# kakaobrain/rq-vae-transformer

Measured on NVIDIA H100. Metric: 256x256 images/sec (ImageNet 1.4B RQ-Transformer, 8x8x4 codes, K=16384, top-k 1024, sample+decode), higher is better.
Workload: dtype fp16

## Files before the change

rq-vae-transformer_b200/csrc/conv_tc.cu:

```cuda
#include <cstdlib>

#include "kernels.h"
#include "tc_common.cuh"

namespace rqb {

struct ConvTcParams {
    int B, H, W, Cin, Cout;
    int ks;
    int stride;
    int TW, TH, NB;
    int tiles_x, tiles_y, tiles_b, n_tiles_n;
    const float* bias;
    const float* residual;
    float* out;
    int out_nchw;
    void* out16;
    int gelu, fmt;
    int64_t m_rows;
    double* gn_part;
    int gn_chunks;
};

constexpr int CT_THREADS = 288;
// ... 222 lines not shown
    const int grid = total < n_sm ? total : n_sm;
    conv_tc_kernel<BN, STAGES, PASSES><<<grid, CT_THREADS, smem, st>>>(tmA, tmB, tmAlo, tmBlo, p);
    return check_launch("conv_tc");
}

constexpr int C3_HALO_BYTES = 10 * 10 * 2 * 128;

template <int BN>
__device__ __forceinline__ void c3_mma_kblock(float (&acc)[BN / 2], uint32_t a, uint32_t b, bool first) {
    constexpr int B_BYTES = BN * 64 * 2;
    constexpr uint32_t SBO = 10 * 128;
#pragma unroll
    for (int j = 0; j < 4; j++)
        tc::Wgmma<BN, 0>::mma(acc, tc::gmma_desc_k128(a + C3_HALO_BYTES + j * 32, SBO), tc::gmma_desc_k128(b + j * 32),
                              (!first || j > 0) ? 1u : 0u);
#pragma unroll
    for (int j = 0; j < 4; j++)
        tc::Wgmma<BN, 0>::mma(acc, tc::gmma_desc_k128(a + j * 32, SBO), tc::gmma_desc_k128(b + B_BYTES + j * 32), 1u);
#pragma unroll
    for (int j = 0; j < 4; j++)
        tc::Wgmma<BN, 0>::mma(acc, tc::gmma_desc_k128(a + j * 32, SBO), tc::gmma_desc_k128(b + j * 32), 1u);
}

template <int BM, int STAGES, int SLOT_BYTES, int HALO_BYTES>
__device__ __forceinline__ void c3_produce(const CUtensorMap* tmA, const CUtensorMap* tmB, const CUtensorMap* tmAlo, const CUtensorMap* tmBlo,
                                           const ConvTcParams& p, uint8_t* smem, uint8_t* wst, uint64_t* full, uint64_t* empty,
                                           uint64_t* hfull, uint64_t* hempty) {
    constexpr int NOPS = 2;
    constexpr int B_BYTES = BM * 64 * 2;
    constexpr int STAGE_BYTES = NOPS * B_BYTES;
    const int cslabs = p.Cin / 64;
    const int total = p.tiles_x * p.tiles_y * p.tiles_b * p.n_tiles_n;
    const uint32_t halo_tx = NOPS * 10 * (p.TH + 2) * p.NB * 128;
    uint32_t it = 0, hit = 0;
    for (int tile = blockIdx.x; tile < total; tile += gridDim.x) {
        const int nt = tile % p.n_tiles_n, mt = tile / p.n_tiles_n;
        const int tx = mt % p.tiles_x, ty = (mt / p.tiles_x) % p.tiles_y, tb = mt / (p.tiles_x * p.tiles_y);
        const int x0 = tx * 8, y0 = ty * p.TH, b0 = tb * p.NB;
        for (int sl = 0; sl < cslabs; sl++, hit++) {
            const int c0 = sl * 64;
            for (int tap = 0; tap < 9; tap++, it++) {
                const int s = it % STAGES;
                tc::mbar_wait(&empty[s], ((it / STAGES) & 1) ^ 1);
                tc::mbar_expect_tx(&full[s], STAGE_BYTES);
                uint8_t* w = wst + s * STAGE_BYTES;
                tc::tma_load_2d(w, tmB, &full[s], tap * p.Cin + c0, nt * BM, tc::L2_EVICT_LAST);
                tc::tma_load_2d(w + B_BYTES, tmBlo, &full[s], tap * p.Cin + c0, nt * BM, tc::L2_EVICT_LAST);
                if (tap == 0) {
                    const int h = hit % 2;
                    tc::mbar_wait(&hempty[h], ((hit / 2) & 1) ^ 1);
                    tc::mbar_expect_tx(&hfull[h], halo_tx);
                    uint8_t* a = smem + h * SLOT_BYTES;
                    tc::tma_load_4d(a, tmA, &hfull[h], c0, x0 - 1, y0 - 1, b0, tc::L2_EVICT_NORMAL);
                    tc::tma_load_4d(a + HALO_BYTES, tmAlo, &hfull[h], c0, x0 - 1, y0 - 1, b0, tc::L2_EVICT_NORMAL);
                }
            }
        }
    }
}

template <int BN, int STAGES>
__global__ void __launch_bounds__(CT_THREADS, 1)
conv3x3_tc_kernel(const __grid_constant__ CUtensorMap tmA, const __grid_constant__ CUtensorMap tmB,
                  const __grid_constant__ CUtensorMap tmAlo, const __grid_constant__ CUtensorMap tmBlo, ConvTcParams p) {
    constexpr int B_BYTES = BN * 64 * 2;
    constexpr int NOPS = 2;
    constexpr int HSLOTS = 2;
    constexpr int SLOT_BYTES = NOPS * C3_HALO_BYTES;
    constexpr int STAGE_BYTES = NOPS * B_BYTES;
    constexpr int CW = BN < 32 ? BN : 32;
// ... 98 lines not shown
template <int TH, int NB>
__device__ __forceinline__ void c3w_mma_kblock(float (&acc)[C3wTile<TH, NB>::NP / 2], const uint32_t (&fh)[4][4],
                                               const uint32_t (&fl)[4][4], uint32_t x, bool first) {
    constexpr int NI = C3wTile<TH, NB>::NI, HALO = C3wTile<TH, NB>::HALO;
    constexpr uint32_t SBO = 10 * 128, IMG = (TH + 2) * 10 * 128;
    auto mma = [&acc](const uint32_t (&a)[4], uint32_t xa, uint32_t accumulate) {
#pragma unroll
        for (int b = 0; b < NB; b++)
            tc::WgmmaRA<NI>::mma(*reinterpret_cast<float(*)[NI / 2]>(&acc[b * (NI / 2)]), a, tc::gmma_desc_k128(xa + b * IMG, SBO),
                                 accumulate);
    };
#pragma unroll
    for (int j = 0; j < 4; j++) mma(fh[j], x + HALO + j * 32, (!first || j > 0) ? 1u : 0u);
#pragma unroll
    for (int j = 0; j < 4; j++) mma(fl[j], x + j * 32, 1u);
#pragma unroll
    for (int j = 0; j < 4; j++) mma(fh[j], x + j * 32, 1u);
}

__device__ __forceinline__ void ldsm_x4(uint32_t (&r)[4], uint32_t addr) {
    asm volatile("ldmatrix.sync.aligned.m8n8.x4.shared.b16 {%0,%1,%2,%3}, [%4];" : "=r"(r[0]), "=r"(r[1]), "=r"(r[2]), "=r"(r[3]) : "r"(addr));
}

template <int TH, int NB, int STAGES>
__global__ void __launch_bounds__(C3W_THREADS, 1)
conv3x3_wreg_kernel(const __grid_constant__ CUtensorMap tmA, const __grid_constant__ CUtensorMap tmB,
                    const __grid_constant__ CUtensorMap tmAlo, const __grid_constant__ CUtensorMap tmBlo, ConvTcParams p) {
    using T = C3wTile<TH, NB>;
    constexpr int NOPS = 2;
    constexpr int SLOT_BYTES = NOPS * T::HALO;
    constexpr int B_BYTES = 128 * 128;
    constexpr int STAGE_BYTES = NOPS * B_BYTES;
    extern __shared__ uint8_t smem_raw[];
    uint8_t* smem = reinterpret_cast<uint8_t*>((reinterpret_cast<uintptr_t>(smem_raw) + 1023) & ~uintptr_t(1023));
    uint8_t* wst = smem + 2 * SLOT_BYTES;
    float* stage = reinterpret_cast<float*>(wst + STAGES * STAGE_BYTES);
    float2* gnred = reinterpret_cast<float2*>(stage + 32 * C3W_SP);
    uint64_t* full = reinterpret_cast<uint64_t*>(gnred + 256);
    uint64_t* empty = full + STAGES;
    uint64_t* hfull = empty + STAGES;
    uint64_t* hempty = hfull + 2;

    const int warp = threadIdx.x >> 5, lane = threadIdx.x & 31;
    const int nkb = 9 * (p.Cin / 64);
    const int total = p.tiles_x * p.tiles_y * p.tiles_b * p.n_tiles_n;

    if (warp == 8 && lane == 0) {
        tc::prefetch_tmap(&tmA);
        tc::prefetch_tmap(&tmB);
        for (int s = 0; s < STAGES; s++) { tc::mbar_init(&full[s], 1); tc::mbar_init(&empty[s], 8); }
        for (int h = 0; h < 2; h++) { tc::mbar_init(&hfull[h], 1); tc::mbar_init(&hempty[h], 8); }
        tc::fence_barrier_init();
    }
    __syncthreads();

    if (warp >= 8) {
        tc::setmaxnreg_dec<C3W_REGS_PRODUCER>();
        if (warp == 8 && lane == 0)
            c3_produce<128, STAGES, SLOT_BYTES, T::HALO>(&tmA, &tmB, &tmAlo, &tmBlo, p, smem, wst, full, empty, hfull, hempty);
        return;
    }
    tc::setmaxnreg_inc<C3W_REGS_CONSUMER>();

    const int wg = warp >> 2;
    const uint32_t lofs = (64 * wg + 16 * (warp & 3) + (lane & 7) + 8 * ((lane >> 3) & 1)) * 128 + (((lane >> 4) ^ (lane & 7)) << 4);
    const uint32_t halo0 = tc::smem_u32(smem), wst0 = tc::smem_u32(wst);

    float acc[T::NP / 2];
#pragma unroll
    for (int i = 0; i < T::NP / 2; i++) acc[i] = 0.f;
    uint32_t frag[2][2][4][4];
    uint32_t it = 0, hit = 0;
    auto kblock = [&](int kb, uint32_t (&fr)[2][4][4]) {
        const int tap = kb % 9;
        if (tap == 0) tc::mbar_wait(&hfull[hit % 2], (hit / 2) & 1);
        const int s = it % STAGES;
        tc::mbar_wait(&full[s], (it / STAGES) & 1);
        const uint32_t w = wst0 + s * STAGE_BYTES + lofs;
#pragma unroll
        for (int j = 0; j < 4; j++) {
            ldsm_x4(fr[0][j], w ^ (32 * j));
            ldsm_x4(fr[1][j], (w + B_BYTES) ^ (32 * j));
        }
        const uint32_t x = halo0 + (hit % 2) * SLOT_BYTES + ((tap / 3) * 10 + tap % 3) * 128;
        tc::wgmma_fence();
        c3w_mma_kblock<TH, NB>(acc, fr[0], fr[1], x, kb == 0);
        tc::wgmma_commit();
        __syncwarp();
        if (lane == 0) tc::mbar_arrive(&empty[s]);
        tc::wgmma_wait<1>();
        if (tap == 0 && kb > 0 && lane == 0) tc::mbar_arrive(&hempty[(hit - 1) % 2]);
        it++;
        if (tap == 8) hit++;
    };
    for (int tile = blockIdx.x; tile < total; tile += gridDim.x) {
        for (int kb = 0; kb < nkb; kb += 2) {
            kblock(kb, frag[0]);
            if (kb + 1 < nkb) kblock(kb + 1, frag[1]);
        }
        tc::wgmma_wait<0>();
        tc::acc_fence(acc);
        if (lane == 0) tc::mbar_arrive(&hempty[(hit - 1) % 2]);

        const int nt = tile % p.n_tiles_n, mt = tile / p.n_tiles_n;
        const int tx = mt % p.tiles_x, ty = (mt / p.tiles_x) % p.tiles_y, tb = mt / (p.tiles_x * p.tiles_y);
        const int srow = 2 * (lane & 3), scol = 64 * wg + 16 * (warp & 3) + (lane >> 2);
        const int n0 = nt * 128 + 4 * lane;
#pragma unroll
        for (int c = 0; c < T::NP / 32; c++) {
#pragma unroll
            for (int jj = 0; jj < 4; jj++)
#pragma unroll
                for (int i = 0; i < 4; i++)
                    stage[(8 * jj + srow + (i & 1)) * C3W_SP + scol + 8 * (i >> 1)] = acc[4 * (4 * c + jj) + i];
            tc::bar_sync(1, 256);
            const int x = tx * 8 + warp, y0 = ty * TH + (4 * c) % TH, b = tb * NB + (4 * c) / TH;
            const int64_t off = (((int64_t)b * p.H + y0) * p.W + x) * p.Cout + n0;
            const int rs = p.W * p.Cout;
            const float4 bb = *reinterpret_cast<const float4*>(p.bias + n0);
            float4 v[4];
            unsigned valid = 0;
#pragma unroll
            for (int r = 0; r < 4; r++) {
                if (x < p.W && y0 + r < p.H && b < p.B) valid |= 1u << r;
                const float4 q = *reinterpret_cast<const float4*>(stage + (8 * r + warp) * C3W_SP + 4 * lane);
                v[r] = make_float4(q.x + bb.x, q.y + bb.y, q.z + bb.z, q.w + bb.w);
            }
            if (p.out_nchw) {
                const int64_t cs = (int64_t)p.H * p.W;
#pragma unroll
                for (int r = 0; r < 4; r++)
                    if (valid >> r & 1) {
                        float* o = p.out + (((int64_t)b * p.Cout + n0) * p.H + y0 + r) * p.W + x;
                        o[0] = v[r].x; o[cs] = v[r].y; o[2 * cs] = v[r].z; o[3 * cs] = v[r].w;
                    }
            } else {
                if (p.residual) {
#pragma unroll
                    for (int r = 0; r < 4; r++)
                        if (valid >> r & 1) {
                            const float4 rr = *reinterpret_cast<const float4*>(p.residual + off + r * rs);
                            v[r].x += rr.x; v[r].y += rr.y; v[r].z += rr.z; v[r].w += rr.w;
                        }
                }
#pragma unroll
                for (int r = 0; r < 4; r++)
                    if (valid >> r & 1) *reinterpret_cast<float4*>(p.out + off + r * rs) = v[r];
            }
            const int cl = p.Cout >> 7;
            if (p.gn_part != nullptr) {
                float s1 = 0.f, s2 = 0.f;
#pragma unroll
                for (int r = 0; r < 4; r++)
                    if (valid >> r & 1) {
                        s1 += (v[r].x + v[r].y) + (v[r].z + v[r].w);
                        s2 += fmaf(v[r].x, v[r].x, v[r].y * v[r].y) + fmaf(v[r].z, v[r].z, v[r].w * v[r].w);
                    }
                for (int m = 1; m < cl; m <<= 1) {
                    s1 += __shfl_xor_sync(0xffffffffu, s1, m);
                    s2 += __shfl_xor_sync(0xffffffffu, s2, m);
                }
                gnred[warp * 32 + lane] = make_float2(s1, s2);
            }
            tc::bar_sync(1, 256);
            if (p.gn_part != nullptr && warp == 0 && (lane & (cl - 1)) == 0) {
                float s1 = 0.f, s2 = 0.f;
#pragma unroll
                for (int w = 0; w < 8; w++) {
                    const float2 q = gnred[w * 32 + lane];
                    s1 += q.x;
                    s2 += q.y;
                }
                const int chunk = (ty * p.tiles_x + tx) * (TH / 4) + c % (TH / 4);
                double* o = p.gn_part + (((int64_t)b * p.gn_chunks + chunk) * 32 + n0 / (4 * cl)) * 2;
                if (b < p.B) { o[0] = (double)s1; o[1] = (double)s2; }
            }
        }
    }
}

template <int TH, int NB, int STAGES>
static int launch_conv3x3_wreg_t(const CUtensorMap& tmA, const CUtensorMap& tmB, const CUtensorMap& tmAlo, const CUtensorMap& tmBlo,
                                 const ConvTcParams& p, int n_sm, cudaStream_t st) {
    constexpr int NOPS = 2;
    constexpr size_t smem = (size_t)2 * NOPS * C3wTile<TH, NB>::HALO + (size_t)STAGES * NOPS * 128 * 128 + 32 * C3W_SP * 4 + 256 * 8 + 1024 + 256;
    static_assert(smem <= 227 * 1024, "conv3x3_wreg: shared memory budget");
    RQB_ENSURE_SMEM(smem, conv3x3_wreg_kernel<TH, NB, STAGES>);
    const int total = p.tiles_x * p.tiles_y * p.tiles_b * p.n_tiles_n;
    const int grid = total < n_sm ? total : n_sm;
    conv3x3_wreg_kernel<TH, NB, STAGES><<<grid, C3W_THREADS, smem, st>>>(tmA, tmB, tmAlo, tmBlo, p);
    return check_launch("conv3x3_wreg");
}

static int sm_count() {
    static int n = 0;
    if (!n) {
        int dev = 0;
        cudaGetDevice(&dev);
        cudaDeviceGetAttribute(&n, cudaDevAttrMultiProcessorCount, dev);
        if (n <= 0) n = 132;
    }
    return n;
}

bool conv_tc_supported(int H, int W, int Cin, int Cout, int ks, int stride, int in_nchw, int out_nchw) {
    if ((stride != 1 && !(stride == 2 && ks == 3)) || in_nchw || (ks != 1 && ks != 3)) return false;
    if (Cin % 64 != 0) return false;
    if (Cout != 3 && Cout % 128 != 0 && Cout != 64) return false;
    if (!out_nchw && Cout % 16 != 0) return false;
    auto pow2 = [](int v) { return v > 0 && (v & (v - 1)) == 0; };
    return pow2(H) && pow2(W);
}

static bool conv3x3_wreg(int Cout, int ks, int stride) { return ks == 3 && stride == 1 && Cout % 128 == 0; }

static void conv_tile(int H, int W, int Cout, int ks, int stride, int& TW, int& TH, int& NB) {
    if (ks == 3 && stride == 1) {
        TW = 8;
        TH = conv3x3_wreg(Cout, ks, stride) && H >= 32 ? 32 : (H > 8 ? 16 : 8);
        NB = TH == 8 ? 2 : 1;
    } else {
        TW = W < 16 ? W : 16;
        TH = (128 / TW) < H ? (128 / TW) : H;
        NB = 128 / (TW * TH);
    }
}

bool conv_tc_gn_fusable(int H, int W, int Cout, int ks, int stride) {
    int TW, TH, NB;
    conv_tile(H, W, Cout, ks, stride, TW, TH, NB);
    const int cg = Cout / 32;
    return Cout % 32 == 0 && (cg == 4 || cg == 8 || cg == 16) && W % TW == 0 && H % TH == 0 && TW * TH >= 32 && (H * W) % 32 == 0;
}

int launch_conv_tc(const void* X16, const void* W16, const void* X16lo, const void* W16lo, const float* bias,
                   const float* residual, float* out, int B, int H, int W, int Cin, int Cout, int ks, int out_nchw,
                   cudaStream_t st, int stride, double* gn_part) {
    if (X16lo == nullptr || W16lo == nullptr) return fail(RQB200_EINVAL, "conv_tc: the lo halves X16lo and W16lo are required");
    if (!out_nchw && Cout % 16 != 0) return fail(RQB200_EINVAL, "conv_tc: an NHWC output needs Cout % 16 == 0");
    if (out_nchw && residual != nullptr) return fail(RQB200_EINVAL, "conv_tc: an NCHW output takes no residual");
    ConvTcParams p = {};
    p.B = B; p.H = H; p.W = W; p.Cin = Cin; p.Cout = Cout; p.ks = ks; p.stride = stride;
    conv_tile(H, W, Cout, ks, stride, p.TW, p.TH, p.NB);
    const bool c3 = ks == 3 && stride == 1;
    if (!c3 && p.TW * p.TH * p.NB != 128) return fail(RQB200_EINVAL, "conv_tc: feature map extent must be a power of two");
    p.tiles_x = (int)ceil_div(W, p.TW); p.tiles_y = (int)ceil_div(H, p.TH); p.tiles_b = (int)ceil_div(B, p.NB);
    const int BN = Cout <= 16 ? 16 : (Cout % 256 == 0 && !c3 ? 256 : (Cout % 128 == 0 ? 128 : 64));
    p.n_tiles_n = (int)ceil_div(Cout, BN);
    p.bias = bias; p.residual = residual; p.out = out; p.out_nchw = out_nchw;
    if (gn_part != nullptr) {
        if (!conv_tc_gn_fusable(H, W, Cout, ks, stride) || out_nchw)
            return fail(RQB200_EINVAL, "conv_tc: GroupNorm statistics cannot be fused for this shape");
        p.gn_part = gn_part;
        p.gn_chunks = H * W / 32;
    }
    CUtensorMap tmA, tmB, tmAlo, tmBlo;
    RQB_TRY(make_tmap_2d(&tmB, W16, 1, (uint64_t)ks * ks * Cin, (uint64_t)Cout, (uint64_t)ks * ks * Cin * 2, 64, (uint32_t)BN));
    RQB_TRY(make_tmap_2d(&tmBlo, W16lo, 1, (uint64_t)ks * ks * Cin, (uint64_t)Cout, (uint64_t)ks * ks * Cin * 2, 64, (uint32_t)BN));
    const int n_sm = sm_count();
    if (c3) {
        RQB_TRY(make_tmap_4d_nhwc(&tmA, X16, (uint64_t)Cin, (uint64_t)W, (uint64_t)H, (uint64_t)B, 64, (uint32_t)p.TW + 2,
                                  (uint32_t)p.TH + 2, (uint32_t)p.NB, 1));
        RQB_TRY(make_tmap_4d_nhwc(&tmAlo, X16lo, (uint64_t)Cin, (uint64_t)W, (uint64_t)H, (uint64_t)B, 64, (uint32_t)p.TW + 2,
                                  (uint32_t)p.TH + 2, (uint32_t)p.NB, 1));
        if (conv3x3_wreg(Cout, ks, stride)) {
            if (p.TH == 32) return launch_conv3x3_wreg_t<32, 1, 1>(tmA, tmB, tmAlo, tmBlo, p, n_sm, st);
            if (p.TH == 16) return launch_conv3x3_wreg_t<16, 1, 3>(tmA, tmB, tmAlo, tmBlo, p, n_sm, st);
            return launch_conv3x3_wreg_t<8, 2, 3>(tmA, tmB, tmAlo, tmBlo, p, n_sm, st);
        }
        return BN == 16 ? launch_conv3x3_tc_t<16, 8>(tmA, tmB, tmAlo, tmBlo, p, n_sm, st)
                        : launch_conv3x3_tc_t<64, 4>(tmA, tmB, tmAlo, tmBlo, p, n_sm, st);
    }
    RQB_TRY(make_tmap_4d_nhwc(&tmA, X16, (uint64_t)Cin, (uint64_t)W * stride, (uint64_t)H * stride, (uint64_t)B, 64, (uint32_t)p.TW,
                              (uint32_t)p.TH, (uint32_t)p.NB, (uint32_t)stride));
    RQB_TRY(make_tmap_4d_nhwc(&tmAlo, X16lo, (uint64_t)Cin, (uint64_t)W * stride, (uint64_t)H * stride, (uint64_t)B, 64,
                              (uint32_t)p.TW, (uint32_t)p.TH, (uint32_t)p.NB, (uint32_t)stride));
    switch (BN) {
        case 16: return launch_conv_tc_t<16, 5, 3>(tmA, tmB, tmAlo, tmBlo, p, n_sm, st);
        case 64: return launch_conv_tc_t<64, 4, 3>(tmA, tmB, tmAlo, tmBlo, p, n_sm, st);
        case 128: return launch_conv_tc_t<128, 3, 3>(tmA, tmB, tmAlo, tmBlo, p, n_sm, st);
        default: return launch_conv_tc_t<256, 2, 3>(tmA, tmB, tmAlo, tmBlo, p, n_sm, st);
    }
}

int launch_rows_gemm_tc(const void* X16, const void* W16, const float* bias, const float* residual, float* out_f32, void* out_16,
                        int gelu, int fmt, int64_t M, int N_out, int K, cudaStream_t st) {
    if (N_out % 128 != 0 || K % 64 != 0 || M < 1 || (out_f32 == nullptr) == (out_16 == nullptr) || bias == nullptr)
        return fail(RQB200_EINVAL, "rows_gemm_tc: need N_out % 128 == 0, K % 64 == 0, a bias and exactly one output");
    ConvTcParams p = {};
    p.B = (int)ceil_div(M, 128); p.H = 8; p.W = 16; p.Cin = K; p.Cout = N_out; p.ks = 1; p.stride = 1;
    p.TW = 16; p.TH = 8; p.NB = 1;
// ... 119 lines not shown
    return check_launch("gn_apply_f16");
}

int launch_cast_f16(const float* X, void* Y16, void* Y16lo, int B, int H, int W, int C, int upsample, cudaStream_t st) {
    if (C % 4 != 0) return fail(RQB200_EINVAL, "cast_f16: C % 4 != 0");
    int64_t total4 = (int64_t)B * H * W * C / 4 * (upsample ? 4 : 1);
    int gx = (int)std::min<int64_t>(ceil_div(total4, 256), sm_count() * 16);
    cast_f16_kernel<<<gx, 256, 0, st>>>(X, (__half*)Y16, (__half*)Y16lo, B, H, W, C, upsample);
    return check_launch("cast_f16");
}

}

extern "C" int rqb200_dbg_conv_tc(const void* X16, const void* W16, const void* X16lo, const void* W16lo, const float* bias,
                                  const float* residual, float* out, int B, int H, int W, int Cin, int Cout, int ks, int out_nchw,
                                  void* stream) {
    return rqb200_dbg_conv_tc_gn(X16, W16, X16lo, W16lo, bias, residual, out, nullptr, B, H, W, Cin, Cout, ks, out_nchw, stream);
}

extern "C" int rqb200_dbg_conv_tc_gn(const void* X16, const void* W16, const void* X16lo, const void* W16lo, const float* bias,
                                     const float* residual, float* out, double* gn_part, int B, int H, int W, int Cin, int Cout, int ks,
                                     int out_nchw, void* stream) {
    const int stride = (out_nchw >> 8) > 1 ? (out_nchw >> 8) : 1;
    if (!rqb::conv_tc_supported(H, W, Cin, Cout, ks, stride, 0, out_nchw & 1)) return rqb::fail(RQB200_EINVAL, "conv_tc: unsupported shape");
    if (out_nchw & 2) return rqb::fail(RQB200_EINVAL, "conv_tc: bf16 operands are not supported (fp16 only)");
    return rqb::launch_conv_tc(X16, W16, X16lo, W16lo, bias, residual, out, B, H, W, Cin, Cout, ks, out_nchw & 1, (cudaStream_t)stream,
                               stride, gn_part);
}

extern "C" int rqb200_dbg_rows_gemm(const void* X16, const void* W16, const float* bias, const float* residual, float* out_f32,
                                    void* out_16, int gelu, int fmt, int64_t M, int N_out, int K, void* stream) {
    return rqb::launch_rows_gemm_tc(X16, W16, bias, residual, out_f32, out_16, gelu, fmt, M, N_out, K, (cudaStream_t)stream);
}
```

rq-vae-transformer_b200/csrc/core.cu:

```cuda
#include "common.cuh"

namespace rqb {
static thread_local std::string g_err;
thread_local int64_t g_launches = 0;
void set_error(const std::string& msg) { g_err = msg; }
int fail(int code, const std::string& msg) {
    g_err = msg;
    return code;
}
}

extern "C" {
const char* rqb200_last_error(void) { return rqb::g_err.c_str(); }
int rqb200_version(void) { return 115; }
int rqb200_device_count(void) {
    int n = 0;
    if (cudaGetDeviceCount(&n) != cudaSuccess) { cudaGetLastError(); return 0; }
    return n;
}
}
```

rq-vae-transformer_b200/csrc/kernels.h:

```cpp
#pragma once
#include <cuda.h>

#include "common.cuh"

namespace rqb {
constexpr int RQ_MAX_TABLES = 16;
struct RqTables {
    const float* cb[RQ_MAX_TABLES];
    int K[RQ_MAX_TABLES];
    int n;
    __host__ __device__ __forceinline__ int of(int depth) const { return n == 1 ? 0 : depth; }
};
int make_rq_tables(RqTables* out, const float* const* cb_host, const int32_t* K_host, int n);

int launch_rq_quantize(const float* x, const RqTables& tabs, int64_t N, int C, int D, int64_t* codes, float* quant_list,
                       float* resid_out, cudaStream_t st, int form = 0);
bool rq_quantize2_supported(int64_t N, const RqTables& tabs, int C);
int launch_rq_quantize2(const float* x, const RqTables& tabs, int64_t N, int C, int D, int64_t* codes, float* quant_list,
                        float* resid_out, cudaStream_t st);
int launch_rq_embed(const int64_t* codes, const RqTables& tabs, int64_t N, int D, int C, float* out, bool sum, cudaStream_t st);
int launch_sample(const float* logits, const float* q, int B, int V, float temperature, int top_k, float top_p,
                  int64_t* out_idx, const int64_t* force, int64_t out_stride, cudaStream_t st, int algo = 1, int cfg_n = 0,
                  float cfg_s = 0.f, const uint8_t* keep = nullptr);
int launch_logprob_rows(const float* lg, int64_t ld, int V, int64_t rows, const int64_t* tgt, int64_t tgt_stride, float* out,
// ... 13 lines not shown
int launch_cond_token(const int64_t* cond, const float* cond_emb, const float* pos_cond, int B, int cond_len, int vocab_cond,
                      int E, int Tn, float* X, cudaStream_t st);
int launch_head_cumsum(const int64_t* codes, const float* cb, int64_t cb_dstride, int B, int HW, int D, int K, int C, int j, int d,
                       float* out, cudaStream_t st, bool last_only = false);
int launch_row_add(const float* in, int64_t in_row_stride, int64_t in_off, const float* pos, int B, int E, float* out,
                   cudaStream_t st);
struct ConvGeom {
    int B, Hi, Wi, Cin;
    int Ho, Wo, Cout;
    int KH, KW, stride;
    int pad;
    int upsample;
    int out_nchw;
    int in_nchw;
};
ConvGeom vae_conv_geom(int B, int H, int W, int Cin, int Cout, int ks, int stride, int upsample, int in_nchw, int out_nchw);
int launch_conv(const float* X, const void* W, int wdtype, const float* bias, const float* R, float* Y, const ConvGeom& g,
                cudaStream_t st);
int launch_groupnorm_silu(const float* X, const float* gamma, const float* beta, float* Y, double* stats_ws, int B, int HW,
                          int C, int silu, cudaStream_t st);
int launch_vae_attn(const float* qkv, float* out, int B, int HW, int C, cudaStream_t st);
size_t groupnorm_ws_doubles(int B, int HW);
int launch_gn_stats(const float* X, double* stats_ws, int B, int HW, int C, cudaStream_t st);
bool conv_tc_supported(int H, int W, int Cin, int Cout, int ks, int stride, int in_nchw, int out_nchw);
int launch_conv_tc(const void* X16, const void* W16, const void* X16lo, const void* W16lo, const float* bias,
                   const float* residual, float* out, int B, int H, int W, int Cin, int Cout, int ks, int out_nchw,
                   cudaStream_t st, int stride = 1, double* gn_part = nullptr);
bool conv_tc_gn_fusable(int H, int W, int Cout, int ks, int stride);
int launch_rows_gemm_tc(const void* X16, const void* W16, const float* bias, const float* residual, float* out_f32, void* out_16,
                        int gelu, int fmt, int64_t M, int N_out, int K, cudaStream_t st);
int launch_groupnorm_f16(const float* X, const float* gamma, const float* beta, void* Y16, void* Y16lo, double* stats_ws, int B,
                         int HW, int C, int silu, cudaStream_t st, int fused_chunks = 0);
int launch_cast_f16(const float* X, void* Y16, void* Y16lo, int B, int H, int W, int C, int upsample, cudaStream_t st);
int make_tmap_4d_nhwc(CUtensorMap* out, const void* base, uint64_t C, uint64_t W, uint64_t H, uint64_t B, uint32_t box_c,
                      uint32_t box_w, uint32_t box_h, uint32_t box_b, uint32_t stride = 1);

enum GemmTcMode { GT_F32 = 0, GT_H16 = 1, GT_H16_GELU = 2, GT_PARTIAL = 3 };
struct GemmTcParams {
    int N_out, K, B, splits, mode;
    int fmt;
    const float* bias;
    float bias_scale;
    const float* residual;
    int64_t ld_res, res_row_stride;
    const int* res_row_ptr;
    int res_div;
    void* out;
    int64_t ld_out;
    float* partial;
    long long* trace;
};
// ... 62 lines not shown
```

rq-vae-transformer_b200/csrc/vae_engine.cu:

```cuda
#include <string>
#include <unordered_map>
#include <vector>

#include "kernels.h"

struct VTensor {
    const void* ptr;
    int dtype;
    int64_t numel;
};

struct rqb200_vae {
    rqb200_vae_config cfg;
    std::unordered_map<std::string, VTensor> t;
    bool finalized = false;
    bool fast_ok = false;
    bool enc_fast = false;
    bool gn_fuse = true;
    int64_t last_launches = 0;
    int64_t max_act = 0;
    int64_t max_gn_hw = 0;
    rqb::RqTables codebooks{};
};

// ... 15 lines not shown
    double* gn_ws;
    std::string missing;
    __half* h16[2] = {nullptr, nullptr};
    __half* l16[2] = {nullptr, nullptr};
    float* zq = nullptr;
    bool fast = false;

    const float* stats_buf = nullptr;
    int stats_chunks = 0;

    const VTensor* get(const std::string& k, int64_t numel) {
        auto it = h->t.find(k);
        if (it == h->t.end() || it->second.numel != numel) {
            if (missing.empty()) missing = k + (it == h->t.end() ? " (missing)" : " (wrong size)");
            return nullptr;
        }
        return &it->second;
    }
    void note_act(int64_t hw, int64_t c) { if (hw * c > h->max_act) h->max_act = hw * c; }

    int operand(const float* x, int H, int W, int C, int slot, int upsample, Operand* o) {
        *o = fast ? Operand{nullptr, slot, upsample, 0} : Operand{x, -1, upsample, 0};
        if (!fast || dry) return 0;
        return launch_cast_f16(x, h16[slot], l16[slot], B, H, W, C, upsample, st);
    }
    int norm(const std::string& name, const float* in, float* out, int HW, int C, int silu, Operand* o) {
        const VTensor* g = get(name + ".weight", C);
        const VTensor* b = get(name + ".bias", C);
        if (HW > h->max_gn_hw) h->max_gn_hw = HW;
        note_act(HW, C);
        *o = fast ? Operand{nullptr, 0, 0, 0} : Operand{out, -1, 0, 0};
        if (dry || !g || !b) return 0;
        if (!fast) return launch_groupnorm_silu(in, (const float*)g->ptr, (const float*)b->ptr, out, gn_ws, B, HW, C, silu, st);
        const int fused = (in == stats_buf) ? stats_chunks : 0;
        stats_buf = nullptr;
        return launch_groupnorm_f16(in, (const float*)g->ptr, (const float*)b->ptr, h16[0], l16[0], gn_ws, B, HW, C, silu, st, fused);
    }
    int conv(const std::string& name, const Operand& in, float* out, const float* resid, int H, int W, int Cin, int Cout, int ks,
             int stride, bool feeds_gn, int out_nchw) {
        const ConvGeom g = vae_conv_geom(B, H, W, Cin, Cout, ks, stride, in.upsample, in.nchw, out_nchw);
        const int Ho = g.Ho, Wo = g.Wo;
        const int64_t wn = (int64_t)Cout * ks * ks * Cin;
        const VTensor* w = get(name + ".weight", wn);
        const VTensor* b = get(name + ".bias", Cout);
        const VTensor* wl = in.slot < 0 ? nullptr : get(name + ".weight_lo", wn);
        note_act((int64_t)Ho * Wo, Cout);
        if (dry || !w || !b) return 0;
        if (in.slot < 0) return launch_conv(in.x, w->ptr, w->dtype, (const float*)b->ptr, resid, out, g, st);
        if (!wl) return 0;
        if (w->dtype != RQB200_F16 || wl->dtype != RQB200_F16)
            return fail(RQB200_ESTATE, "vae fast tier: conv weights and their lo halves must be fp16: " + name);
        const bool fuse = feeds_gn && h->gn_fuse && !out_nchw && conv_tc_gn_fusable(Ho, Wo, Cout, ks, stride);
        stats_buf = fuse ? out : nullptr;
        stats_chunks = fuse ? Ho * Wo / 32 : 0;
        return launch_conv_tc(h16[in.slot], w->ptr, l16[in.slot], wl->ptr, (const float*)b->ptr, resid, out, B, Ho, Wo, Cin, Cout, ks, out_nchw, st,
                              stride, fuse ? gn_ws : nullptr);
    }

    int resblock(const std::string& p, int& cur, int H, int W, int Cin, int Cout) {
        const int a = (cur + 1) & 3, b = (cur + 2) & 3, c = (cur + 3) & 3;
        Operand x;
        RQB_TRY(norm(p + ".norm1", buf[cur], buf[a], H * W, Cin, 1, &x));
        RQB_TRY(conv(p + ".conv1", x, buf[b], nullptr, H, W, Cin, Cout, 3, 1, true, 0));
        RQB_TRY(norm(p + ".norm2", buf[b], buf[a], H * W, Cout, 1, &x));
        const float* res = buf[cur];
        if (Cin != Cout) {
            Operand s;
            RQB_TRY(operand(buf[cur], H, W, Cin, 1, 0, &s));
            RQB_TRY(conv(p + ".nin_shortcut", s, buf[c], nullptr, H, W, Cin, Cout, 1, 1, false, 0));
            res = buf[c];
        }
        RQB_TRY(conv(p + ".conv2", x, buf[b], res, H, W, Cout, Cout, 3, 1, true, 0));
        cur = b;
        return 0;
    }
    int attnblock(const std::string& p, int& cur, int H, int W, int C) {
        const int a = (cur + 1) & 3, b = (cur + 2) & 3, c = (cur + 3) & 3;
        Operand x;
        RQB_TRY(norm(p + ".norm", buf[cur], buf[a], H * W, C, 0, &x));
// ... 258 lines not shown
```

rq-vae-transformer_b200/rqvae/models/rqvae/rqvae.py:

```python
import ctypes as C
import os

import torch
from torch import nn
from torch.nn import functional as F

from ... import _native as N
from ..interfaces import Stage1Model
from .modules import Decoder, Encoder, ResnetBlock
from .quantizations import RQBottleneck


class RQVAE(Stage1Model):
    def __init__(self, *, embed_dim=64, n_embed=512, decay=0.99, loss_type="mse", latent_loss_weight=0.25,
                 bottleneck_type="rq", ddconfig=None, checkpointing=False, **kwargs):
        super().__init__()
        assert loss_type in ("mse", "l1")
        ddconfig = dict(ddconfig)
        self.ddconfig = ddconfig
        self.encoder = Encoder(**ddconfig)
        self.decoder = Decoder(**ddconfig)
        if bottleneck_type != "rq":
            raise ValueError("invalid 'bottleneck_type' (must be 'rq')")
        self.quantizer = RQBottleneck(latent_shape=kwargs["latent_shape"], code_shape=kwargs["code_shape"], n_embed=n_embed,
                                      decay=decay, shared_codebook=kwargs["shared_codebook"],
                                      restart_unused_codes=kwargs["restart_unused_codes"])
        self.code_shape = kwargs["code_shape"]
        self.embed_dim = embed_dim
        self.quant_conv = nn.Conv2d(ddconfig["z_channels"], embed_dim, 1)
        self.post_quant_conv = nn.Conv2d(embed_dim, ddconfig["z_channels"], 1)
        self.loss_type, self.latent_loss_weight = loss_type, latent_loss_weight
        self.precision = None
        self._eng = {}
# ... 37 lines not shown
        cfg = N.VaeConfig()
        cfg.ch, cfg.n_levels, cfg.num_res_blocks = dd["ch"], len(dd["ch_mult"]), dd["num_res_blocks"]
        for i, m in enumerate(dd["ch_mult"]):
            cfg.ch_mult[i] = m
        cfg.n_attn_res = len(dd["attn_resolutions"])
        for i, r in enumerate(dd["attn_resolutions"]):
            cfg.attn_resolutions[i] = r
        cfg.resolution, cfg.z_channels, cfg.embed_dim = dd["resolution"], dd["z_channels"], self.embed_dim
        cfg.in_channels, cfg.out_ch = dd["in_channels"], dd["out_ch"]
        cfg.codebook_size, cfg.depth, cfg.mode = self.quantizer.n_embed[0], self.code_shape[-1], mode
        if os.environ.get("RQB200_GN_FUSE", "1") == "0":
            cfg.mode |= 0x100
        handle = L.rqb200_vae_create(C.byref(cfg))
        if not handle:
            raise N.NativeError("rqb200_vae_create: " + L.rqb200_last_error().decode())
        wdt = torch.float16 if mode == N.MODE_FAST else torch.float32
        keep = {}

        def reg(name, t):
            t = t.detach().contiguous()
            keep[name] = t
            N.check(L.rqb200_vae_set_tensor(handle, name.encode(), N.ptr(t), N.dtype_code(t), t.numel()), "vae_set_tensor")

        def reg_conv(name, w_oihw):
            w = w_oihw.detach().permute(0, 2, 3, 1).contiguous().float()
            if mode == N.MODE_FAST and not name.startswith("encoder.conv_in"):
                hi = w.to(torch.float16)
                reg(name, hi)
                reg(name + "_lo", (w - hi.float()).to(torch.float16))
            else:
                reg(name, w)

        sd = {k: v for k, v in self.state_dict().items()}
        for k, v in sd.items():
            if not (k.startswith("encoder.") or k.startswith("decoder.") or k.startswith("quant_conv") or
                    k.startswith("post_quant_conv")):
                continue
            N.require_cuda(v)
            if v.dim() == 4:
                if k.endswith((".q.weight", ".k.weight", ".v.weight")):
                    continue
                reg_conv(k, v)
            elif k.endswith((".q.bias", ".k.bias", ".v.bias")):
                continue
            else:
                reg(k, v.float())
        for k in [k for k in sd if k.endswith(".q.weight")]:
            base = k[:-len(".q.weight")]
            w = torch.cat([sd[base + ".q.weight"], sd[base + ".k.weight"], sd[base + ".v.weight"]], 0)
            b = torch.cat([sd[base + ".q.bias"], sd[base + ".k.bias"], sd[base + ".v.bias"]], 0)
            reg_conv(base + ".qkv.weight", w)
            reg(base + ".qkv.bias", b.float())
# ... 101 lines not shown
```

Measured before the change: 197.3.

## Fold nearest-neighbor upsample into 3x3 conv via four 2x2 phase kernels

```diff
diff --git a/rq-vae-transformer_b200/csrc/conv_tc.cu b/rq-vae-transformer_b200/csrc/conv_tc.cu
--- a/rq-vae-transformer_b200/csrc/conv_tc.cu
+++ b/rq-vae-transformer_b200/csrc/conv_tc.cu
@@ -268,30 +268,41 @@
         tc::Wgmma<BN, 0>::mma(acc, tc::gmma_desc_k128(a + j * 32, SBO), tc::gmma_desc_k128(b + j * 32), 1u);
 }
 
-template <int BM, int STAGES, int SLOT_BYTES, int HALO_BYTES>
+template <bool UP>
+__device__ __forceinline__ void c3_item(const ConvTcParams& p, int tile, int& ph, int& nt, int& tx, int& ty, int& tb) {
+    ph = UP ? tile % 4 : 0;
+    const int nm = UP ? tile / 4 : tile;
+    nt = nm % p.n_tiles_n;
+    const int mt = nm / p.n_tiles_n;
+    tx = mt % p.tiles_x; ty = (mt / p.tiles_x) % p.tiles_y; tb = mt / (p.tiles_x * p.tiles_y);
+}
+
+template <int BM, int STAGES, int SLOT_BYTES, int HALO_BYTES, bool UP = false>
 __device__ __forceinline__ void c3_produce(const CUtensorMap* tmA, const CUtensorMap* tmB, const CUtensorMap* tmAlo, const CUtensorMap* tmBlo,
                                            const ConvTcParams& p, uint8_t* smem, uint8_t* wst, uint64_t* full, uint64_t* empty,
                                            uint64_t* hfull, uint64_t* hempty) {
     constexpr int NOPS = 2;
     constexpr int B_BYTES = BM * 64 * 2;
     constexpr int STAGE_BYTES = NOPS * B_BYTES;
+    constexpr int NT = UP ? 4 : 9;
     const int cslabs = p.Cin / 64;
-    const int total = p.tiles_x * p.tiles_y * p.tiles_b * p.n_tiles_n;
+    const int total = p.tiles_x * p.tiles_y * p.tiles_b * p.n_tiles_n * (UP ? 4 : 1);
     const uint32_t halo_tx = NOPS * 10 * (p.TH + 2) * p.NB * 128;
     uint32_t it = 0, hit = 0;
     for (int tile = blockIdx.x; tile < total; tile += gridDim.x) {
-        const int nt = tile % p.n_tiles_n, mt = tile / p.n_tiles_n;
-        const int tx = mt % p.tiles_x, ty = (mt / p.tiles_x) % p.tiles_y, tb = mt / (p.tiles_x * p.tiles_y);
+        int ph, nt, tx, ty, tb;
+        c3_item<UP>(p, tile, ph, nt, tx, ty, tb);
         const int x0 = tx * 8, y0 = ty * p.TH, b0 = tb * p.NB;
+        const int wrow = ph * p.Cout + nt * BM;
         for (int sl = 0; sl < cslabs; sl++, hit++) {
             const int c0 = sl * 64;
-            for (int tap = 0; tap < 9; tap++, it++) {
+            for (int tap = 0; tap < NT; tap++, it++) {
                 const int s = it % STAGES;
                 tc::mbar_wait(&empty[s], ((it / STAGES) & 1) ^ 1);
                 tc::mbar_expect_tx(&full[s], STAGE_BYTES);
                 uint8_t* w = wst + s * STAGE_BYTES;
-                tc::tma_load_2d(w, tmB, &full[s], tap * p.Cin + c0, nt * BM, tc::L2_EVICT_LAST);
-                tc::tma_load_2d(w + B_BYTES, tmBlo, &full[s], tap * p.Cin + c0, nt * BM, tc::L2_EVICT_LAST);
+                tc::tma_load_2d(w, tmB, &full[s], tap * p.Cin + c0, wrow, tc::L2_EVICT_LAST);
+                tc::tma_load_2d(w + B_BYTES, tmBlo, &full[s], tap * p.Cin + c0, wrow, tc::L2_EVICT_LAST);
                 if (tap == 0) {
                     const int h = hit % 2;
                     tc::mbar_wait(&hempty[h], ((hit / 2) & 1) ^ 1);
@@ -436,7 +447,7 @@
     asm volatile("ldmatrix.sync.aligned.m8n8.x4.shared.b16 {%0,%1,%2,%3}, [%4];" : "=r"(r[0]), "=r"(r[1]), "=r"(r[2]), "=r"(r[3]) : "r"(addr));
 }
 
-template <int TH, int NB, int STAGES>
+template <int TH, int NB, int STAGES, bool UP>
 __global__ void __launch_bounds__(C3W_THREADS, 1)
 conv3x3_wreg_kernel(const __grid_constant__ CUtensorMap tmA, const __grid_constant__ CUtensorMap tmB,
                     const __grid_constant__ CUtensorMap tmAlo, const __grid_constant__ CUtensorMap tmBlo, ConvTcParams p) {
@@ -455,9 +466,10 @@
     uint64_t* hfull = empty + STAGES;
     uint64_t* hempty = hfull + 2;
 
+    constexpr int NT = UP ? 4 : 9;
     const int warp = threadIdx.x >> 5, lane = threadIdx.x & 31;
-    const int nkb = 9 * (p.Cin / 64);
-    const int total = p.tiles_x * p.tiles_y * p.tiles_b * p.n_tiles_n;
+    const int nkb = NT * (p.Cin / 64);
+    const int total = p.tiles_x * p.tiles_y * p.tiles_b * p.n_tiles_n * (UP ? 4 : 1);
 
     if (warp == 8 && lane == 0) {
         tc::prefetch_tmap(&tmA);
@@ -471,14 +483,15 @@
     if (warp >= 8) {
         tc::setmaxnreg_dec<C3W_REGS_PRODUCER>();
         if (warp == 8 && lane == 0)
-            c3_produce<128, STAGES, SLOT_BYTES, T::HALO>(&tmA, &tmB, &tmAlo, &tmBlo, p, smem, wst, full, empty, hfull, hempty);
+            c3_produce<128, STAGES, SLOT_BYTES, T::HALO, UP>(&tmA, &tmB, &tmAlo, &tmBlo, p, smem, wst, full, empty, hfull, hempty);
         return;
     }
     tc::setmaxnreg_inc<C3W_REGS_CONSUMER>();
 
     const int wg = warp >> 2;
     const uint32_t lofs = (64 * wg + 16 * (warp & 3) + (lane & 7) + 8 * ((lane >> 3) & 1)) * 128 + (((lane >> 4) ^ (lane & 7)) << 4);
-    const uint32_t halo0 = tc::smem_u32(smem), wst0 = tc::smem_u32(wst);
+    const uint32_t wst0 = tc::smem_u32(wst);
+    uint32_t halo0 = tc::smem_u32(smem);
 
     float acc[T::NP / 2];
 #pragma unroll
@@ -486,7 +499,7 @@
     uint32_t frag[2][2][4][4];
     uint32_t it = 0, hit = 0;
     auto kblock = [&](int kb, uint32_t (&fr)[2][4][4]) {
-        const int tap = kb % 9;
+        const int tap = kb % NT;
         if (tap == 0) tc::mbar_wait(&hfull[hit % 2], (hit / 2) & 1);
         const int s = it % STAGES;
         tc::mbar_wait(&full[s], (it / STAGES) & 1);
@@ -496,7 +509,7 @@
             ldsm_x4(fr[0][j], w ^ (32 * j));
             ldsm_x4(fr[1][j], (w + B_BYTES) ^ (32 * j));
         }
-        const uint32_t x = halo0 + (hit % 2) * SLOT_BYTES + ((tap / 3) * 10 + tap % 3) * 128;
+        const uint32_t x = halo0 + (hit % 2) * SLOT_BYTES + (UP ? (tap >> 1) * 10 + (tap & 1) : (tap / 3) * 10 + tap % 3) * 128;
         tc::wgmma_fence();
         c3w_mma_kblock<TH, NB>(acc, fr[0], fr[1], x, kb == 0);
         tc::wgmma_commit();
@@ -505,9 +518,10 @@
         tc::wgmma_wait<1>();
         if (tap == 0 && kb > 0 && lane == 0) tc::mbar_arrive(&hempty[(hit - 1) % 2]);
         it++;
-        if (tap == 8) hit++;
+        if (tap == NT - 1) hit++;
     };
     for (int tile = blockIdx.x; tile < total; tile += gridDim.x) {
+        if (UP) halo0 = tc::smem_u32(smem) + (((tile & 3) >> 1) * 10 + (tile & 1)) * 128;
         for (int kb = 0; kb < nkb; kb += 2) {
             kblock(kb, frag[0]);
             if (kb + 1 < nkb) kblock(kb + 1, frag[1]);
@@ -516,8 +530,11 @@
         tc::acc_fence(acc);
         if (lane == 0) tc::mbar_arrive(&hempty[(hit - 1) % 2]);
 
-        const int nt = tile % p.n_tiles_n, mt = tile / p.n_tiles_n;
-        const int tx = mt % p.tiles_x, ty = (mt / p.tiles_x) % p.tiles_y, tb = mt / (p.tiles_x * p.tiles_y);
+        int ph, nt, tx, ty, tb;
+        c3_item<UP>(p, tile, ph, nt, tx, ty, tb);
+        const int Hs = p.H >> UP, Ws = p.W >> UP;
+        const int x = tx * 8 + warp;
+        const int pofs = UP ? (ph >> 1) * p.W + 2 * x + (ph & 1) : x;
         const int srow = 2 * (lane & 3), scol = 64 * wg + 16 * (warp & 3) + (lane >> 2);
         const int n0 = nt * 128 + 4 * lane;
 #pragma unroll
@@ -528,19 +545,19 @@
                 for (int i = 0; i < 4; i++)
                     stage[(8 * jj + srow + (i & 1)) * C3W_SP + scol + 8 * (i >> 1)] = acc[4 * (4 * c + jj) + i];
             tc::bar_sync(1, 256);
-            const int x = tx * 8 + warp, y0 = ty * TH + (4 * c) % TH, b = tb * NB + (4 * c) / TH;
-            const int64_t off = (((int64_t)b * p.H + y0) * p.W + x) * p.Cout + n0;
-            const int rs = p.W * p.Cout;
+            const int y0 = ty * TH + (4 * c) % TH, b = tb * NB + (4 * c) / TH;
+            const int64_t off = (((int64_t)b * p.H + (y0 << UP)) * p.W + pofs) * p.Cout + n0;
+            const int rs = (p.W * p.Cout) << UP;
             const float4 bb = *reinterpret_cast<const float4*>(p.bias + n0);
             float4 v[4];
             unsigned valid = 0;
 #pragma unroll
             for (int r = 0; r < 4; r++) {
-                if (x < p.W && y0 + r < p.H && b < p.B) valid |= 1u << r;
+                if (x < Ws && y0 + r < Hs && b < p.B) valid |= 1u << r;
                 const float4 q = *reinterpret_cast<const float4*>(stage + (8 * r + warp) * C3W_SP + 4 * lane);
                 v[r] = make_float4(q.x + bb.x, q.y + bb.y, q.z + bb.z, q.w + bb.w);
             }
-            if (p.out_nchw) {
+            if (!UP && p.out_nchw) {
                 const int64_t cs = (int64_t)p.H * p.W;
 #pragma unroll
                 for (int r = 0; r < 4; r++)
@@ -585,7 +602,7 @@
                     s1 += q.x;
                     s2 += q.y;
                 }
-                const int chunk = (ty * p.tiles_x + tx) * (TH / 4) + c % (TH / 4);
+                const int chunk = ((ty * p.tiles_x + tx) * (TH / 4) + c % (TH / 4)) * (UP ? 4 : 1) + ph;
                 double* o = p.gn_part + (((int64_t)b * p.gn_chunks + chunk) * 32 + n0 / (4 * cl)) * 2;
                 if (b < p.B) { o[0] = (double)s1; o[1] = (double)s2; }
             }
@@ -593,16 +610,16 @@
     }
 }
 
-template <int TH, int NB, int STAGES>
+template <int TH, int NB, int STAGES, bool UP>
 static int launch_conv3x3_wreg_t(const CUtensorMap& tmA, const CUtensorMap& tmB, const CUtensorMap& tmAlo, const CUtensorMap& tmBlo,
                                  const ConvTcParams& p, int n_sm, cudaStream_t st) {
     constexpr int NOPS = 2;
     constexpr size_t smem = (size_t)2 * NOPS * C3wTile<TH, NB>::HALO + (size_t)STAGES * NOPS * 128 * 128 + 32 * C3W_SP * 4 + 256 * 8 + 1024 + 256;
     static_assert(smem <= 227 * 1024, "conv3x3_wreg: shared memory budget");
-    RQB_ENSURE_SMEM(smem, conv3x3_wreg_kernel<TH, NB, STAGES>);
-    const int total = p.tiles_x * p.tiles_y * p.tiles_b * p.n_tiles_n;
+    RQB_ENSURE_SMEM(smem, conv3x3_wreg_kernel<TH, NB, STAGES, UP>);
+    const int total = p.tiles_x * p.tiles_y * p.tiles_b * p.n_tiles_n * (UP ? 4 : 1);
     const int grid = total < n_sm ? total : n_sm;
-    conv3x3_wreg_kernel<TH, NB, STAGES><<<grid, C3W_THREADS, smem, st>>>(tmA, tmB, tmAlo, tmBlo, p);
+    conv3x3_wreg_kernel<TH, NB, STAGES, UP><<<grid, C3W_THREADS, smem, st>>>(tmA, tmB, tmAlo, tmBlo, p);
     return check_launch("conv3x3_wreg");
 }
 
@@ -617,7 +634,10 @@
     return n;
 }
 
-bool conv_tc_supported(int H, int W, int Cin, int Cout, int ks, int stride, int in_nchw, int out_nchw) {
+bool conv_tc_supported(int H, int W, int Cin, int Cout, int ks, int stride, int in_nchw, int out_nchw, int upsample) {
+    if (upsample)
+        return ks == 3 && stride == 1 && !in_nchw && !out_nchw && Cin % 64 == 0 && Cout % 128 == 0 && H >= 2 && W >= 2 && H % 2 == 0 &&
+               W % 2 == 0;
     if ((stride != 1 && !(stride == 2 && ks == 3)) || in_nchw || (ks != 1 && ks != 3)) return false;
     if (Cin % 64 != 0) return false;
     if (Cout != 3 && Cout % 128 != 0 && Cout != 64) return false;
@@ -640,47 +660,58 @@
     }
 }
 
-bool conv_tc_gn_fusable(int H, int W, int Cout, int ks, int stride) {
+bool conv_tc_gn_fusable(int H, int W, int Cout, int ks, int stride, int upsample) {
+    const int Hs = upsample ? H / 2 : H, Ws = upsample ? W / 2 : W;
     int TW, TH, NB;
-    conv_tile(H, W, Cout, ks, stride, TW, TH, NB);
+    conv_tile(Hs, Ws, Cout, ks, stride, TW, TH, NB);
     const int cg = Cout / 32;
-    return Cout % 32 == 0 && (cg == 4 || cg == 8 || cg == 16) && W % TW == 0 && H % TH == 0 && TW * TH >= 32 && (H * W) % 32 == 0;
+    return Cout % 32 == 0 && (cg == 4 || cg == 8 || cg == 16) && Ws % TW == 0 && Hs % TH == 0 && TW * TH >= 32 && (H * W) % 32 == 0 &&
+           (!upsample || (H % 2 == 0 && W % 2 == 0));
 }
 
 int launch_conv_tc(const void* X16, const void* W16, const void* X16lo, const void* W16lo, const float* bias,
                    const float* residual, float* out, int B, int H, int W, int Cin, int Cout, int ks, int out_nchw,
-                   cudaStream_t st, int stride, double* gn_part) {
+                   cudaStream_t st, int stride, double* gn_part, int upsample) {
     if (X16lo == nullptr || W16lo == nullptr) return fail(RQB200_EINVAL, "conv_tc: the lo halves X16lo and W16lo are required");
+    if (upsample && !conv_tc_supported(H, W, Cin, Cout, ks, stride, 0, out_nchw, 1))
+        return fail(RQB200_EINVAL, "conv_tc: the upsample form needs a 3x3 stride-1 conv, Cout % 128 == 0, NHWC output and an even extent");
     if (!out_nchw && Cout % 16 != 0) return fail(RQB200_EINVAL, "conv_tc: an NHWC output needs Cout % 16 == 0");
     if (out_nchw && residual != nullptr) return fail(RQB200_EINVAL, "conv_tc: an NCHW output takes no residual");
     ConvTcParams p = {};
     p.B = B; p.H = H; p.W = W; p.Cin = Cin; p.Cout = Cout; p.ks = ks; p.stride = stride;
-    conv_tile(H, W, Cout, ks, stride, p.TW, p.TH, p.NB);
+    const int Hs = upsample ? H / 2 : H, Ws = upsample ? W / 2 : W;
+    conv_tile(Hs, Ws, Cout, ks, stride, p.TW, p.TH, p.NB);
     const bool c3 = ks == 3 && stride == 1;
     if (!c3 && p.TW * p.TH * p.NB != 128) return fail(RQB200_EINVAL, "conv_tc: feature map extent must be a power of two");
-    p.tiles_x = (int)ceil_div(W, p.TW); p.tiles_y = (int)ceil_div(H, p.TH); p.tiles_b = (int)ceil_div(B, p.NB);
+    p.tiles_x = (int)ceil_div(Ws, p.TW); p.tiles_y = (int)ceil_div(Hs, p.TH); p.tiles_b = (int)ceil_div(B, p.NB);
     const int BN = Cout <= 16 ? 16 : (Cout % 256 == 0 && !c3 ? 256 : (Cout % 128 == 0 ? 128 : 64));
     p.n_tiles_n = (int)ceil_div(Cout, BN);
     p.bias = bias; p.residual = residual; p.out = out; p.out_nchw = out_nchw;
     if (gn_part != nullptr) {
-        if (!conv_tc_gn_fusable(H, W, Cout, ks, stride) || out_nchw)
+        if (!conv_tc_gn_fusable(H, W, Cout, ks, stride, upsample) || out_nchw)
             return fail(RQB200_EINVAL, "conv_tc: GroupNorm statistics cannot be fused for this shape");
         p.gn_part = gn_part;
         p.gn_chunks = H * W / 32;
     }
     CUtensorMap tmA, tmB, tmAlo, tmBlo;
-    RQB_TRY(make_tmap_2d(&tmB, W16, 1, (uint64_t)ks * ks * Cin, (uint64_t)Cout, (uint64_t)ks * ks * Cin * 2, 64, (uint32_t)BN));
-    RQB_TRY(make_tmap_2d(&tmBlo, W16lo, 1, (uint64_t)ks * ks * Cin, (uint64_t)Cout, (uint64_t)ks * ks * Cin * 2, 64, (uint32_t)BN));
+    const uint64_t wk = (uint64_t)(upsample ? 4 : ks * ks) * Cin, wrows = (uint64_t)(upsample ? 4 : 1) * Cout;
+    RQB_TRY(make_tmap_2d(&tmB, W16, 1, wk, wrows, wk * 2, 64, (uint32_t)BN));
+    RQB_TRY(make_tmap_2d(&tmBlo, W16lo, 1, wk, wrows, wk * 2, 64, (uint32_t)BN));
     const int n_sm = sm_count();
     if (c3) {
-        RQB_TRY(make_tmap_4d_nhwc(&tmA, X16, (uint64_t)Cin, (uint64_t)W, (uint64_t)H, (uint64_t)B, 64, (uint32_t)p.TW + 2,
+        RQB_TRY(make_tmap_4d_nhwc(&tmA, X16, (uint64_t)Cin, (uint64_t)Ws, (uint64_t)Hs, (uint64_t)B, 64, (uint32_t)p.TW + 2,
                                   (uint32_t)p.TH + 2, (uint32_t)p.NB, 1));
-        RQB_TRY(make_tmap_4d_nhwc(&tmAlo, X16lo, (uint64_t)Cin, (uint64_t)W, (uint64_t)H, (uint64_t)B, 64, (uint32_t)p.TW + 2,
+        RQB_TRY(make_tmap_4d_nhwc(&tmAlo, X16lo, (uint64_t)Cin, (uint64_t)Ws, (uint64_t)Hs, (uint64_t)B, 64, (uint32_t)p.TW + 2,
                                   (uint32_t)p.TH + 2, (uint32_t)p.NB, 1));
+        if (upsample) {
+            if (p.TH == 32) return launch_conv3x3_wreg_t<32, 1, 1, true>(tmA, tmB, tmAlo, tmBlo, p, n_sm, st);
+            if (p.TH == 16) return launch_conv3x3_wreg_t<16, 1, 3, true>(tmA, tmB, tmAlo, tmBlo, p, n_sm, st);
+            return launch_conv3x3_wreg_t<8, 2, 3, true>(tmA, tmB, tmAlo, tmBlo, p, n_sm, st);
+        }
         if (conv3x3_wreg(Cout, ks, stride)) {
-            if (p.TH == 32) return launch_conv3x3_wreg_t<32, 1, 1>(tmA, tmB, tmAlo, tmBlo, p, n_sm, st);
-            if (p.TH == 16) return launch_conv3x3_wreg_t<16, 1, 3>(tmA, tmB, tmAlo, tmBlo, p, n_sm, st);
-            return launch_conv3x3_wreg_t<8, 2, 3>(tmA, tmB, tmAlo, tmBlo, p, n_sm, st);
+            if (p.TH == 32) return launch_conv3x3_wreg_t<32, 1, 1, false>(tmA, tmB, tmAlo, tmBlo, p, n_sm, st);
+            if (p.TH == 16) return launch_conv3x3_wreg_t<16, 1, 3, false>(tmA, tmB, tmAlo, tmBlo, p, n_sm, st);
+            return launch_conv3x3_wreg_t<8, 2, 3, false>(tmA, tmB, tmAlo, tmBlo, p, n_sm, st);
         }
         return BN == 16 ? launch_conv3x3_tc_t<16, 8>(tmA, tmB, tmAlo, tmBlo, p, n_sm, st)
                         : launch_conv3x3_tc_t<64, 4>(tmA, tmB, tmAlo, tmBlo, p, n_sm, st);
@@ -846,10 +877,12 @@
                                      const float* residual, float* out, double* gn_part, int B, int H, int W, int Cin, int Cout, int ks,
                                      int out_nchw, void* stream) {
     const int stride = (out_nchw >> 8) > 1 ? (out_nchw >> 8) : 1;
-    if (!rqb::conv_tc_supported(H, W, Cin, Cout, ks, stride, 0, out_nchw & 1)) return rqb::fail(RQB200_EINVAL, "conv_tc: unsupported shape");
+    const int upsample = (out_nchw >> 2) & 1;
+    if (!rqb::conv_tc_supported(H, W, Cin, Cout, ks, stride, 0, out_nchw & 1, upsample))
+        return rqb::fail(RQB200_EINVAL, "conv_tc: unsupported shape");
     if (out_nchw & 2) return rqb::fail(RQB200_EINVAL, "conv_tc: bf16 operands are not supported (fp16 only)");
     return rqb::launch_conv_tc(X16, W16, X16lo, W16lo, bias, residual, out, B, H, W, Cin, Cout, ks, out_nchw & 1, (cudaStream_t)stream,
-                               stride, gn_part);
+                               stride, gn_part, upsample);
 }
 
 extern "C" int rqb200_dbg_rows_gemm(const void* X16, const void* W16, const float* bias, const float* residual, float* out_f32,
diff --git a/rq-vae-transformer_b200/csrc/core.cu b/rq-vae-transformer_b200/csrc/core.cu
--- a/rq-vae-transformer_b200/csrc/core.cu
+++ b/rq-vae-transformer_b200/csrc/core.cu
@@ -12,7 +12,7 @@
 
 extern "C" {
 const char* rqb200_last_error(void) { return rqb::g_err.c_str(); }
-int rqb200_version(void) { return 115; }
+int rqb200_version(void) { return 116; }
 int rqb200_device_count(void) {
     int n = 0;
     if (cudaGetDeviceCount(&n) != cudaSuccess) { cudaGetLastError(); return 0; }
diff --git a/rq-vae-transformer_b200/csrc/kernels.h b/rq-vae-transformer_b200/csrc/kernels.h
--- a/rq-vae-transformer_b200/csrc/kernels.h
+++ b/rq-vae-transformer_b200/csrc/kernels.h
@@ -59,11 +59,11 @@
 int launch_vae_attn(const float* qkv, float* out, int B, int HW, int C, cudaStream_t st);
 size_t groupnorm_ws_doubles(int B, int HW);
 int launch_gn_stats(const float* X, double* stats_ws, int B, int HW, int C, cudaStream_t st);
-bool conv_tc_supported(int H, int W, int Cin, int Cout, int ks, int stride, int in_nchw, int out_nchw);
+bool conv_tc_supported(int H, int W, int Cin, int Cout, int ks, int stride, int in_nchw, int out_nchw, int upsample = 0);
 int launch_conv_tc(const void* X16, const void* W16, const void* X16lo, const void* W16lo, const float* bias,
                    const float* residual, float* out, int B, int H, int W, int Cin, int Cout, int ks, int out_nchw,
-                   cudaStream_t st, int stride = 1, double* gn_part = nullptr);
-bool conv_tc_gn_fusable(int H, int W, int Cout, int ks, int stride);
+                   cudaStream_t st, int stride = 1, double* gn_part = nullptr, int upsample = 0);
+bool conv_tc_gn_fusable(int H, int W, int Cout, int ks, int stride, int upsample = 0);
 int launch_rows_gemm_tc(const void* X16, const void* W16, const float* bias, const float* residual, float* out_f32, void* out_16,
                         int gelu, int fmt, int64_t M, int N_out, int K, cudaStream_t st);
 int launch_groupnorm_f16(const float* X, const float* gamma, const float* beta, void* Y16, void* Y16lo, double* stats_ws, int B,
diff --git a/rq-vae-transformer_b200/csrc/vae_engine.cu b/rq-vae-transformer_b200/csrc/vae_engine.cu
--- a/rq-vae-transformer_b200/csrc/vae_engine.cu
+++ b/rq-vae-transformer_b200/csrc/vae_engine.cu
@@ -61,7 +61,7 @@
     int operand(const float* x, int H, int W, int C, int slot, int upsample, Operand* o) {
         *o = fast ? Operand{nullptr, slot, upsample, 0} : Operand{x, -1, upsample, 0};
         if (!fast || dry) return 0;
-        return launch_cast_f16(x, h16[slot], l16[slot], B, H, W, C, upsample, st);
+        return launch_cast_f16(x, h16[slot], l16[slot], B, H, W, C, 0, st);
     }
     int norm(const std::string& name, const float* in, float* out, int HW, int C, int silu, Operand* o) {
         const VTensor* g = get(name + ".weight", C);
@@ -79,21 +79,23 @@
              int stride, bool feeds_gn, int out_nchw) {
         const ConvGeom g = vae_conv_geom(B, H, W, Cin, Cout, ks, stride, in.upsample, in.nchw, out_nchw);
         const int Ho = g.Ho, Wo = g.Wo;
-        const int64_t wn = (int64_t)Cout * ks * ks * Cin;
-        const VTensor* w = get(name + ".weight", wn);
+        const bool phases = in.slot >= 0 && in.upsample;
+        const int64_t wn = (int64_t)Cout * (phases ? 16 : ks * ks) * Cin;
+        const std::string wkey = name + (phases ? ".weight_ph" : ".weight");
+        const VTensor* w = get(wkey, wn);
         const VTensor* b = get(name + ".bias", Cout);
-        const VTensor* wl = in.slot < 0 ? nullptr : get(name + ".weight_lo", wn);
+        const VTensor* wl = in.slot < 0 ? nullptr : get(wkey + "_lo", wn);
         note_act((int64_t)Ho * Wo, Cout);
         if (dry || !w || !b) return 0;
         if (in.slot < 0) return launch_conv(in.x, w->ptr, w->dtype, (const float*)b->ptr, resid, out, g, st);
         if (!wl) return 0;
         if (w->dtype != RQB200_F16 || wl->dtype != RQB200_F16)
             return fail(RQB200_ESTATE, "vae fast tier: conv weights and their lo halves must be fp16: " + name);
-        const bool fuse = feeds_gn && h->gn_fuse && !out_nchw && conv_tc_gn_fusable(Ho, Wo, Cout, ks, stride);
+        const bool fuse = feeds_gn && h->gn_fuse && !out_nchw && conv_tc_gn_fusable(Ho, Wo, Cout, ks, stride, phases);
         stats_buf = fuse ? out : nullptr;
         stats_chunks = fuse ? Ho * Wo / 32 : 0;
         return launch_conv_tc(h16[in.slot], w->ptr, l16[in.slot], wl->ptr, (const float*)b->ptr, resid, out, B, Ho, Wo, Cin, Cout, ks, out_nchw, st,
-                              stride, fuse ? gn_ws : nullptr);
+                              stride, fuse ? gn_ws : nullptr, phases);
     }
 
     int resblock(const std::string& p, int& cur, int H, int W, int Cin, int Cout) {
diff --git a/rq-vae-transformer_b200/rqvae/models/rqvae/rqvae.py b/rq-vae-transformer_b200/rqvae/models/rqvae/rqvae.py
--- a/rq-vae-transformer_b200/rqvae/models/rqvae/rqvae.py
+++ b/rq-vae-transformer_b200/rqvae/models/rqvae/rqvae.py
@@ -9,6 +9,14 @@
 from ..interfaces import Stage1Model
 from .modules import Decoder, Encoder, ResnetBlock
 from .quantizations import RQBottleneck
+
+PHASE_TAPS = ((1, 0, 0), (0, 1, 1)), ((1, 1, 0), (0, 0, 1))
+
+
+def upsample_phase_weights(w_oihw):
+    r = torch.tensor(PHASE_TAPS, dtype=torch.float64, device=w_oihw.device)
+    wp = torch.einsum("pak,qbl,oikl->pqoabi", r, r, w_oihw.double())
+    return wp.reshape(4, *wp.shape[2:]).float().contiguous()
 
 
 class RQVAE(Stage1Model):
@@ -92,12 +100,17 @@
             keep[name] = t
             N.check(L.rqb200_vae_set_tensor(handle, name.encode(), N.ptr(t), N.dtype_code(t), t.numel()), "vae_set_tensor")
 
+        def reg_split(name, w):
+            hi = w.to(torch.float16)
+            reg(name, hi)
+            reg(name + "_lo", (w - hi.float()).to(torch.float16))
+
         def reg_conv(name, w_oihw):
             w = w_oihw.detach().permute(0, 2, 3, 1).contiguous().float()
             if mode == N.MODE_FAST and not name.startswith("encoder.conv_in"):
-                hi = w.to(torch.float16)
-                reg(name, hi)
-                reg(name + "_lo", (w - hi.float()).to(torch.float16))
+                reg_split(name, w)
+                if name.endswith(".upsample.conv.weight"):
+                    reg_split(name + "_ph", upsample_phase_weights(w_oihw.detach()))
             else:
                 reg(name, w)
 
```

Measured after the change: 201.8 (median of 6 runs). 1.02x the previous value.
